# pc2/StencilStream

Measured on NVIDIA B200. Metric: GCell-updates/s, higher is better.
Workload: dtype f32

## Files before the change

include/stst_workloads.h:

```cpp
#ifndef STST_WORKLOADS_H
#define STST_WORKLOADS_H

#include <stddef.h>
#include <stdint.h>

#ifdef __cplusplus
extern "C" {
#endif

#define STST_WORKLOADS_ABI_VERSION 3

#define STST_OK 0
#define STST_ERR_UNKNOWN_WORKLOAD (-1)
#define STST_ERR_INVALID_ARGUMENT (-2)
#define STST_ERR_RANGE (-3)
#define STST_ERR_RUNTIME (-4)



typedef struct stst_hotspot_cell {
    float temp;
    float power;
} stst_hotspot_cell;

// ... 108 lines not shown
int stst_grid_max_abs(stst_grid *grid, const stst_field_extent *extents, size_t n, double *out);
int stst_grid_copy_field_to_host(stst_grid *grid, size_t field, void *values, size_t bytes);
int stst_grid_copy_field_from_host(stst_grid *grid, size_t field, const void *values, size_t bytes);


typedef struct stst_update stst_update;

typedef struct stst_update_params {
    const void *transition_function;
    size_t transition_function_bytes;
    const void *halo_value;
    size_t halo_value_bytes;
    size_t iteration_offset;
    size_t n_iterations;
    int blocking;
    int profiling;
    int cuda_device;
    unsigned fused_iterations;
    unsigned tile_rows;
    const int *cuda_devices;
    size_t n_cuda_devices;
} stst_update_params;

typedef struct stst_update_stats {
    size_t n_processed_cells;
    double walltime;
    double kernel_runtime;
    size_t n_launches;
    unsigned fused_iterations, tile_h, tile_w, block_x, block_y, use_tma;
    size_t smem_bytes;
    unsigned passthrough_planes;
    size_t speculation_redos;
    size_t n_slabs;
} stst_update_stats;

int stst_update_create(const char *workload, const stst_update_params *params, stst_update **update);
int stst_update_set_params(stst_update *update, const stst_update_params *params);
int stst_update_apply(stst_update *update, stst_grid *source, stst_grid **result);
int stst_update_get_stats(stst_update *update, stst_update_stats *stats);
int stst_update_destroy(stst_update *update);


typedef struct stst_slab stst_slab;

typedef struct stst_slab_info {
    size_t grid_rows, grid_cols, row_lo, row_hi;
    size_t ghost_rows;
    size_t device_bytes;
    size_t n_launches;
    size_t epoch;
    int device;
    unsigned fused_iterations, tile_h, tile_w, block_x, block_y, use_tma, overlap;
    size_t smem_bytes;
    unsigned passthrough_planes;
} stst_slab_info;

int stst_slab_create(const char *workload, size_t grid_rows, size_t grid_cols, size_t row_lo,
                     size_t row_hi, int device, unsigned fused_iterations, unsigned tile_rows,
                     int overlap, stst_slab **slab);
int stst_slab_destroy(stst_slab *slab);
int stst_slab_get_info(stst_slab *slab, stst_slab_info *info);
int stst_slab_get_ipc_handle(stst_slab *slab, unsigned char handle[64]);
int stst_slab_attach_ipc(stst_slab *slab, int side, const unsigned char handle[64],
                         size_t peer_row_lo, size_t peer_row_hi);
int stst_slab_attach_local(stst_slab *slab, int side, stst_slab *peer);
int stst_slab_use_nccl(stst_slab *slab, void *nccl_comm, int up_rank, int down_rank);
int stst_slab_detach(stst_slab *slab);
// ... 25 lines not shown
```

stencilstream_b200/_native.py:

```python
from __future__ import annotations

import ctypes as C
import os
from pathlib import Path

import numpy as np

PKG = Path(__file__).resolve().parent


class NativeLibraryMissing(RuntimeError):
    pass



class ConwayParams(C.Structure):
    _fields_ = [("reserved", C.c_int32)]


class Jacobi5Params(C.Structure):
    _fields_ = [("coef", C.c_float * 5)]


class Jacobi9Params(C.Structure):
# ... 28 lines not shown

class ConvectionThermalParams(C.Structure):
    _fields_ = [("nx", C.c_uint64), ("ny", C.c_uint64), ("dx", C.c_double), ("dy", C.c_double),
                ("dt", C.c_double), ("DcT", C.c_double)]


class KatParams(C.Structure):
    _fields_ = [("reserved", C.c_int32)]


class WorkloadInfo(C.Structure):
    _fields_ = [("cell_bytes", C.c_size_t), ("params_bytes", C.c_size_t), ("n_planes", C.c_size_t),
                ("stencil_radius", C.c_size_t), ("n_subiterations", C.c_size_t),
                ("bytes_per_cell_iteration", C.c_size_t)]


class UpdateParams(C.Structure):
    _fields_ = [
        ("transition_function", C.c_void_p), ("transition_function_bytes", C.c_size_t),
        ("halo_value", C.c_void_p), ("halo_value_bytes", C.c_size_t),
        ("iteration_offset", C.c_size_t), ("n_iterations", C.c_size_t),
        ("blocking", C.c_int), ("profiling", C.c_int), ("cuda_device", C.c_int),
        ("fused_iterations", C.c_uint), ("tile_rows", C.c_uint),
        ("cuda_devices", C.POINTER(C.c_int)), ("n_cuda_devices", C.c_size_t),
    ]


class UpdateStats(C.Structure):
    _fields_ = [
        ("n_processed_cells", C.c_size_t), ("walltime", C.c_double), ("kernel_runtime", C.c_double),
        ("n_launches", C.c_size_t), ("fused_iterations", C.c_uint), ("tile_h", C.c_uint),
        ("tile_w", C.c_uint), ("block_x", C.c_uint), ("block_y", C.c_uint), ("use_tma", C.c_uint),
        ("smem_bytes", C.c_size_t), ("passthrough_planes", C.c_uint), ("speculation_redos", C.c_size_t),
        ("n_slabs", C.c_size_t),
    ]


class FieldExtent(C.Structure):
    _fields_ = [("field", C.c_size_t), ("rows", C.c_size_t), ("cols", C.c_size_t)]


class DeviceInfo(C.Structure):
    _fields_ = [
        ("sm_count", C.c_int), ("cc_major", C.c_int), ("cc_minor", C.c_int),
        ("max_smem_per_block_optin", C.c_int), ("max_smem_per_sm", C.c_int), ("l2_bytes", C.c_int),
        ("clock_khz", C.c_int), ("total_mem", C.c_size_t), ("free_mem", C.c_size_t),
        ("name", C.c_char * 128),
    ]



CELL_DTYPES = {
    "conway": np.dtype(np.bool_),
    "jacobi5": np.dtype(np.float32),
    "jacobi9": np.dtype(np.float32),
    "jacobi_r2": np.dtype(np.float32),
    "jacobi_r3": np.dtype(np.float32),
    "hotspot": np.dtype([("temp", "<f4"), ("power", "<f4")]),
    "fdtd": np.dtype([(n, "<f4") for n in ("ex", "ey", "hz", "hz_sum", "ca", "cb", "da", "db")]),
    "convection_pt": np.dtype([(n, "<f8") for n in (
        "T", "Pt", "Vx", "Vy", "tau_xx", "tau_yy", "sigma_xy", "dVxd_tau", "dVyd_tau", "ErrV", "ErrP")]),
    "kat": np.dtype([(n, "<i4") for n in ("r", "c", "i_iteration", "i_subiteration", "status")]),
}
CELL_DTYPES["convection_thermal"] = CELL_DTYPES["convection_pt"]
CELL_DTYPES["kat_r2"] = CELL_DTYPES["kat"]


# ... 137 lines not shown
```

stencilstream_b200/csrc/workloads/model.hpp:

```cpp
#pragma once
#include <StencilStream/cuda/StencilUpdate.hpp>
#include <StencilStream/cuda/internal/SlabUpdate.hpp>
#include <stst_workloads.h>

#include "functors.hpp"

#include <algorithm>
#include <cstring>
#include <memory>
#include <stdexcept>
#include <string>
#include <vector>

namespace stst_model {

using namespace stst_workloads;
namespace sc = stencil::cuda;

inline thread_local std::string g_error;

inline int report(int code, std::string message) {
    g_error = std::move(message);
    return code;
}
// ... 102 lines not shown

    UpdateHolder(const char *name, const stst_update_params &p)
        : update(std::make_unique<Update>(convert(p))) {
        workload = name;
    }

    void set_params(const stst_update_params &p) override { update->get_params() = convert(p); }

    GridBase *apply(GridBase &source) override {
        auto *typed = dynamic_cast<GridHolder<Cell> *>(&source);
        if (!typed)
            throw std::invalid_argument("grid belongs to a workload with a different cell type");
        sc::Grid<Cell> result = (*update)(typed->grid);
        return new GridHolder<Cell>(source.workload, result);
    }

    void stats(stst_update_stats &s) override {
        std::memset(&s, 0, sizeof(s));
        s.n_processed_cells = update->get_n_processed_cells();
        s.walltime = update->get_walltime();
        s.kernel_runtime = update->get_kernel_runtime();
        s.n_launches = update->get_n_launches();
        auto const &plan = update->get_last_plan();
        s.fused_iterations = plan.fused_iterations;
        s.tile_h = plan.tile_h;
        s.tile_w = plan.tile_w;
        s.block_x = plan.block_x;
        s.block_y = plan.block_y;
        s.use_tma = plan.use_tma ? 1u : 0u;
        s.smem_bytes = plan.smem_bytes;
        s.passthrough_planes = update->get_passthrough_planes();
        s.speculation_redos = update->get_n_speculation_redos();
        s.n_slabs = update->get_n_slabs();
    }
};

struct SlabBase {
    virtual ~SlabBase() = default;
    const char *workload = nullptr;
    std::vector<void *> ipc_mappings;
    virtual std::size_t cell_bytes() const = 0;
    virtual void info(stst_slab_info &out) = 0;
    virtual void *device_base() = 0;
    virtual int device() const = 0;
    virtual void attach(int side, void *mapped, std::size_t lo, std::size_t hi) = 0;
    virtual void detach() = 0;
    virtual void use_nccl(void *comm, int up_rank, int down_rank) = 0;
    virtual void upload(const void *cells, std::size_t first_row, std::size_t n_rows) = 0;
    virtual void download(void *cells, std::size_t first_row, std::size_t n_rows) = 0;
    virtual void exchange() = 0;
    virtual void max_abs(const stst_field_extent *extents, std::size_t n, double *out) = 0;
    virtual std::size_t field_bytes(std::size_t field) const = 0;
    virtual void download_field(std::size_t field, void *host, std::size_t first_row,
                                std::size_t n_rows) = 0;
    virtual void update(const stst_update_params &p) = 0;
    virtual void synchronize() = 0;
    virtual void record(void *event) = 0;
    virtual void copy_from(SlabBase &other) = 0;
    virtual sc::internal::PlaneSet current_planes() = 0;
    virtual std::size_t ghost() const = 0;
    virtual bool enable_speculation(bool on) = 0;
    virtual void backup() = 0;
    virtual void restore() = 0;
    virtual unsigned take_violations() = 0;
    virtual void drop_passthrough(unsigned planes) = 0;
};
// ... 149 lines not shown
```

stencilstream_b200/include/StencilStream/cuda/StencilUpdate.hpp:

```cpp
#pragma once
#include "../Concepts.hpp"
#include "../Stencil.hpp"
#include "Grid.hpp"
#include "internal/Helpers.hpp"
#include "internal/Launch.hpp"
#include "internal/PassThrough.hpp"
#include "internal/Planner.hpp"
#include "internal/Runtime.hpp"
#include "internal/SlabUpdate.hpp"
#include "internal/TileKernel.hpp"

#include <algorithm>
#include <chrono>
#include <cstdio>
#include <cstdlib>
#include <memory>
#include <string>
#include <vector>

namespace stencil {
namespace cuda {

template <concepts::TransitionFunction F, bool split_cell_structure = false> class StencilUpdate {
  public:
// ... 174 lines not shown
    }

    GridImpl run_passes(GridImpl &source, internal::LaunchPlan const &plan,
                        internal::Speculation const *spec, std::size_t iteration,
                        std::size_t n_iterations, bool source_is_scratch = false) {
        last_plan = plan;
        const std::size_t k = plan.fused_iterations;
        GridImpl swap_a = source.make_similar();
        GridImpl swap_b = source_is_scratch ? source
                          : (n_iterations > k) ? source.make_similar()
                                               : swap_a;
        swap_a.get_storage().allocate_device();
        swap_b.get_storage().allocate_device();
        lap("allocate scratch grids");

        GridImpl *pass_source = &source, *pass_target = &swap_a;
        while (n_iterations > 0) {
            const unsigned n_gens = unsigned(std::min(n_iterations, k));
            launch(plan, pass_source->get_storage(), pass_target->get_storage(), iteration, n_gens,
                   spec);
            iteration += n_gens;
            n_iterations -= n_gens;
            pass_source = pass_target;
            pass_target = (pass_target == &swap_a) ? &swap_b : &swap_a;
        }
        pass_source->get_storage().device_written();
        lap("submit launches");
        return *pass_source;
    }

    internal::LaunchPlan plan_for(internal::GridStorage<Cell> const &source, unsigned single_planes) {
        const internal::LaunchPlan plan = internal::make_plan<F>(
            source.device, unsigned(source.height), unsigned(source.width), params.n_iterations,
            params.fused_iterations, params.tile_rows, single_planes);
        lap("make_plan");
        return plan;
    }

    void lap(const char *what) {
        if (!std::getenv("STST_TRACE"))
            return;
        const auto now = std::chrono::high_resolution_clock::now();
        std::fprintf(stderr, "[stst] %-22s %9.3f ms\n", what,
                     std::chrono::duration<double, std::milli>(now - lap_start).count());
        lap_start = now;
    }


    using Slab = internal::SlabUpdate<F>;

    struct ShardSet {
        ~ShardSet() {
            for (auto &slab : slabs)
                if (slab)
                    slab->synchronize();
        }
        std::vector<int> devices;
        std::size_t grid_h = 0, grid_w = 0;
        unsigned fused_override = 0, tile_rows = 0;
        std::vector<std::unique_ptr<Slab>> slabs;
        std::vector<std::unique_ptr<internal::Event>> done;
        bool speculating = false;
    };

    std::vector<int> resolve_devices() const {
        if (!params.cuda_devices.empty())
            return params.cuda_devices;
// ... 236 lines not shown
```

stencilstream_b200/include/StencilStream/cuda/internal/Launch.hpp:

```cpp
#pragma once
#include "Helpers.hpp"
#include "PassThrough.hpp"
#include "Planner.hpp"
#include "Runtime.hpp"
#include "TileKernel.hpp"

#include <climits>
#include <cstring>
#include <map>
#include <stdexcept>
#include <string>
#include <tuple>

namespace stencil {
namespace cuda {
namespace internal {

struct LaunchRegion {
    int device;
    unsigned grid_h, grid_w;
    int buf_row0;
    std::size_t buf_rows;
    int out_row_lo;
    int out_row_hi;
// ... 5 lines not shown
template <typename Cell> class TensorMapCache {
  public:
    using Layout = CellLayout<Cell>;

    TensorMapSet const &get(PlaneSet const &planes, std::size_t width, std::size_t rows,
                            unsigned box_cols, unsigned box_rows) {
        const Key key{planes.base[0], planes.pitch[0], width, rows, box_cols, box_rows};
        auto it = cache.find(key);
        if (it != cache.end())
            return it->second;
        if (cache.size() >= 64)
            cache.clear();
        TensorMapSet maps{};
        for (std::size_t i = 0; i < Layout::n_planes; i++) {
            STST_RT_CHECK(stst_tensor_map_encode_2d(
                &maps.map[i][0], planes.base[i], int(Layout::plane_bytes(i)), width, rows,
                planes.pitch[i] * Layout::plane_bytes(i), box_cols, box_rows));
        }
        return cache.emplace(key, maps).first->second;
    }

    void clear() { cache.clear(); }

  private:
    using Key = std::tuple<void *, unsigned long long, std::size_t, std::size_t, unsigned, unsigned>;
    std::map<Key, TensorMapSet> cache;
};

template <typename F> struct SweepLauncher {
    using Cell = typename F::Cell;
    using TDV = typename F::TimeDependentValue;
    using Layout = CellLayout<Cell>;
    static constexpr int CW = column_group_width<Cell>();
#if defined(STST_WINDOW_MODE)
    static constexpr int kMode = STST_WINDOW_MODE;
#else
    static constexpr int kMode = sizeof(Cell) <= 8    ? window_rotate
                                 : sizeof(Cell) <= 16 ? window_shift
                                                      : window_reload;
#endif

    static void launch(LaunchPlan const &plan, F const &tf, Cell const &halo_value,
                       PlaneSet const &src, PlaneSet const &dst, HaloPush const *push,
                       LaunchRegion const &region, std::size_t iteration0, unsigned n_gens,
                       TensorMapCache<Cell> &maps_cache, stst_stream_t stream,
                       Speculation const *spec = nullptr) {
#if defined(__CUDACC__)
        constexpr unsigned n_sub = unsigned(F::n_subiterations);
        constexpr unsigned radius = unsigned(F::stencil_radius);
        if (n_gens == 0 || n_gens > plan.fused_iterations || n_gens > max_fused_iterations)
            throw std::invalid_argument("StencilStream-B200: illegal number of fused iterations");
        if (region.out_row_hi <= region.out_row_lo || region.grid_w == 0)
            return;

        SweepGeometry geo{};
        geo.grid_h = region.grid_h;
        geo.grid_w = region.grid_w;
        geo.buf_row0 = region.buf_row0;
        geo.buf_rows = unsigned(region.buf_rows);
        geo.out_row_lo = region.out_row_lo;
        geo.out_row_hi = region.out_row_hi;
        geo.tile_h = region.tile_h ? std::min(region.tile_h, plan.tile_h) : plan.tile_h;
        const bool second = region.out2_row_hi > region.out2_row_lo;
        geo.tile_h = std::min(geo.tile_h, unsigned(region.out_row_hi - region.out_row_lo));
        if (second)
            geo.tile_h = std::min(geo.tile_h, unsigned(region.out2_row_hi - region.out2_row_lo));
        geo.tile_w = plan.tile_w;
        geo.halo = n_gens * n_sub * radius;
        geo.hpad = plan.hpad;
        geo.n_gens = n_gens;
        geo.tiles_x = (geo.grid_w + geo.tile_w - 1) / geo.tile_w;
        geo.use_tma = plan.use_tma ? 1u : 0u;
        geo.push = push ? 1u : 0u;
        geo.inv_block_y = (1u << 24) / plan.block_y + 1u;
        constexpr unsigned all_planes =
            Layout::n_planes >= 32 ? ~0u : ((1u << Layout::n_planes) - 1u);
        unsigned single_planes = 0;
        if (spec) {
            if constexpr (speculation_capable<F>()) {
                for (unsigned q = 0; q < n_sub && q < max_spec_subiterations; q++)
                    geo.keep[q] = spec->probe ? 0u : (spec->keep[q] & all_planes);
                geo.probe = spec->probe ? 1u : 0u;
                geo.spec_flags = spec->flags;
                single_planes = spec->probe ? 0u : spec->single_planes(n_sub, all_planes);
                if (single_planes != plan.single_planes)
                    throw std::logic_error("StencilStream-B200: plan and speculation masks disagree");
// ... 47 lines not shown
                                             cudaGetErrorString(err));
                configured_smem = smem;
            }
            kernel<<<grid, block, smem, static_cast<cudaStream_t>(stream)>>>(
                tf, halo_value, tdvs, src, dst, push ? *push : no_push, *maps, geo);
        };
        static std::size_t configured_smem_per_device[2][64] = {};
        if constexpr (speculation_capable<F>()) {
            if (spec) {
                submit(fused_sweep_kernel<F, CW, kMode, fixed_block_x<Cell>(),
                                          max_threads_per_cta<Cell>(), 1, true>,
                       configured_smem_per_device[1][region.device & 63]);
            } else {
                submit(fused_sweep_kernel<F, CW, kMode, fixed_block_x<Cell>(),
                                          max_threads_per_cta<Cell>(), 1, false>,
                       configured_smem_per_device[0][region.device & 63]);
            }
        } else {
            submit(fused_sweep_kernel<F, CW, kMode, fixed_block_x<Cell>(),
                                      max_threads_per_cta<Cell>(), 1, false>,
                   configured_smem_per_device[0][region.device & 63]);
        }
        cudaError_t err = cudaGetLastError();
        if (err != cudaSuccess)
            throw std::runtime_error(std::string("StencilStream-B200: kernel launch failed: ") +
                                     cudaGetErrorString(err));
#else
        (void)plan, (void)tf, (void)halo_value, (void)src, (void)dst, (void)push, (void)region;
        (void)iteration0, (void)n_gens, (void)maps_cache, (void)stream;
        throw std::runtime_error("StencilStream-B200 must be compiled with nvcc for sm_100a; "
                                 "there is no CPU fallback");
#endif
    }
};

}
}
}
```

stencilstream_b200/include/StencilStream/cuda/internal/Planner.hpp:

```cpp
#pragma once
#include "Helpers.hpp"
#include "Runtime.hpp"
#include "TileKernel.hpp"

#include <algorithm>
#include <cmath>
#include <cstdlib>
#include <stdexcept>
#include <string>

namespace stencil {
namespace cuda {
namespace internal {

struct LaunchPlan {
    unsigned fused_iterations;
    unsigned block_x, block_y;
    unsigned tile_h, tile_w;
    unsigned halo, hpad;
    std::size_t smem_bytes;
    bool use_tma;
    unsigned single_planes;
};

inline long env_long(const char *name, long fallback) {
    const char *v = std::getenv(name);
    return (v && *v) ? std::atol(v) : fallback;
}

inline const stst_device_info &cached_device_info(int device) {
    constexpr int max_devices = 64;
    static stst_device_info infos[max_devices];
    static bool valid[max_devices] = {};
    if (device < 0 || device >= max_devices)
        throw std::invalid_argument("StencilStream-B200: device ordinal out of range");
    if (!valid[device]) {
        STST_RT_CHECK(stst_get_device_info(device, &infos[device]));
        valid[device] = true;
    }
    return infos[device];
}

template <typename Cell> constexpr int column_group_width() {
    if (sizeof(Cell) > 64) {
#if defined(STST_FAT_COLUMN_GROUP_WIDTH)
        return STST_FAT_COLUMN_GROUP_WIDTH;
#else
        return 1;
#endif
    }
    const std::size_t widest = CellLayout<Cell>::max_plane_bytes();
    if (widest >= 16)
        return 1;
    if (widest >= 8)
        return 2;
// ... 5 lines not shown
#endif
    }
#if defined(STST_LIGHT_COLUMN_GROUP_WIDTH)
    if (CellLayout<Cell>::n_planes == 1 && widest == 4)
        return STST_LIGHT_COLUMN_GROUP_WIDTH;
#endif
    return 4;
}

template <typename Cell> constexpr int max_threads_per_cta() {
#if defined(STST_LIGHT_MAX_THREADS)
    if (sizeof(Cell) <= 8)
        return STST_LIGHT_MAX_THREADS;
#endif
    if (sizeof(Cell) > 16 && sizeof(Cell) <= 64) {
#if defined(STST_MID_MAX_THREADS)
        return STST_MID_MAX_THREADS;
#else
        return 384;
#endif
    }
    if (sizeof(Cell) > 64 && column_group_width<Cell>() == 1) {
#if defined(STST_FAT_MAX_THREADS)
        return STST_FAT_MAX_THREADS;
#else
        return 640;
#endif
    }
    return 256;
}

template <typename Cell> constexpr int fixed_block_x() {
    return lane_major_tiles<Cell, column_group_width<Cell>()>() ? 256 / column_group_width<Cell>() : 0;
}

template <typename Cell> constexpr bool tma_capable() {
    using L = CellLayout<Cell>;
    constexpr int cw = column_group_width<Cell>();
    for (std::size_t i = 0; i < L::n_planes; i++) {
        const std::size_t b = L::plane_bytes(i);
        if (!(b == 1 || b == 2 || b == 4 || b == 8))
            return false;
        if ((b * cw * 32) % 16 != 0)
            return false;
    }
    return true;
}

template <typename Cell> constexpr unsigned column_alignment(bool for_tma) {
    using L = CellLayout<Cell>;
    unsigned align = unsigned(column_group_width<Cell>());
    if (for_tma) {
        for (std::size_t i = 0; i < L::n_planes; i++) {
            const unsigned need = unsigned(16 / (L::plane_bytes(i) < 16 ? L::plane_bytes(i) : 16));
            align = need > align ? need : align;
        }
    }
    return align;
}

struct TileShape {
    unsigned halo, hpad, tile_h, tile_w, rows, cols;
    std::size_t smem_bytes;
    double efficiency;
    bool feasible;
};

template <typename Cell>
TileShape shape_for(unsigned k, unsigned n_sub, unsigned radius, unsigned cw, unsigned col_align,
                    unsigned block_x, unsigned tile_rows_override, std::size_t smem_budget,
                    unsigned grid_h, unsigned single_planes = 0) {
    TileShape s{};
    s.halo = k * n_sub * radius;
    s.hpad = (s.halo + col_align - 1) / col_align * col_align;
    s.cols = block_x * cw;
    s.feasible = false;
    if (2 * s.hpad >= s.cols)
        return s;
    s.tile_w = s.cols - 2 * s.hpad;
    const unsigned n_buffers = (k * n_sub > 1) ? 2 : 1;
    const std::size_t per_row = tile_buffer_bytes<Cell>(1, s.cols) +
                                tile_buffer_bytes<Cell>(1, s.cols, single_planes) * (n_buffers - 1);
    const std::size_t usable = smem_budget > 4096 ? smem_budget - 2048 : 0;
    unsigned max_rows = unsigned(std::min<std::size_t>(usable / std::max<std::size_t>(per_row, 1), 256));
    if (max_rows <= 2 * s.halo)
        return s;
    unsigned tile_h = max_rows - 2 * s.halo;
    if (tile_rows_override > 0)
        tile_h = std::min(tile_h, tile_rows_override);
    tile_h = std::min(tile_h, std::max(grid_h, 1u));
    s.tile_h = tile_h;
    s.rows = tile_h + 2 * s.halo;
    s.smem_bytes = tile_smem_bytes<Cell>(s.rows, s.cols, n_buffers, single_planes);
    s.efficiency = double(s.tile_h) * s.tile_w / (double(s.rows) * s.cols);
    s.feasible = s.smem_bytes <= smem_budget;
    return s;
}

template <typename F>
LaunchPlan make_plan(int device, unsigned grid_h, unsigned grid_w, std::size_t n_iterations,
                     unsigned fused_override, unsigned tile_rows_override,
                     unsigned single_planes = 0) {
    using Cell = typename F::Cell;
    using L = CellLayout<Cell>;
    constexpr unsigned cw = unsigned(column_group_width<Cell>());
    constexpr unsigned n_sub = unsigned(F::n_subiterations);
    constexpr unsigned radius = unsigned(F::stencil_radius);

    const stst_device_info &info = cached_device_info(device);
    const std::size_t smem_optin = std::size_t(info.max_smem_per_block_optin);
    const std::size_t smem_sm = std::size_t(info.max_smem_per_sm);

    unsigned block_x = unsigned(env_long("STST_BLOCK_X", 0));
    if (block_x == 0) {
        block_x = (sizeof(Cell) <= 16 || cw == 1) ? 64 : 32;
        if (cw > 4)
            block_x = 32;
        while (block_x > 32 && block_x * cw / 2 >= std::max(grid_w, 1u) + 2 * cw)
            block_x /= 2;
    }
    block_x = std::max(32u, block_x / 32 * 32);
    if (fixed_block_x<Cell>() != 0)
        block_x = unsigned(fixed_block_x<Cell>());
    unsigned block_y = unsigned(env_long("STST_BLOCK_Y", 0));
    if (block_y == 0)
        block_y = std::max(1u, unsigned(max_threads_per_cta<Cell>()) / block_x);
    if (block_x * block_y > unsigned(max_threads_per_cta<Cell>()))
        throw std::invalid_argument("StencilStream-B200: CTA shape exceeds the compiled thread limit");

    if (fused_override == 0)
        fused_override = unsigned(env_long("STST_FUSE", 0));
    if (tile_rows_override == 0)
        tile_rows_override = unsigned(env_long("STST_TILE_ROWS", 0));
    const unsigned ctas_per_sm = unsigned(std::max(1l, env_long("STST_CTAS_PER_SM", 2)));

    const unsigned k_cap = unsigned(
        std::min<std::size_t>(std::max<std::size_t>(n_iterations, 1), max_fused_iterations));

    auto budget_for = [&](unsigned ctas) {
        std::size_t per_cta = smem_sm / ctas;
        per_cta = per_cta > 1024 ? per_cta - 1024 : 0;
        return std::min(per_cta, smem_optin);
    };

    const bool want_tma = tma_capable<Cell>() && env_long("STST_TMA", 1) != 0;
    const unsigned col_align = column_alignment<Cell>(want_tma);

    auto evaluate = [&](unsigned k, unsigned ctas) {
        return shape_for<Cell>(k, n_sub, radius, cw, col_align, block_x, tile_rows_override,
                               budget_for(ctas), grid_h, single_planes);
    };

    unsigned best_k = 0;
    TileShape best{};
    const double hbm_bytes = 2.0 * double(sizeof(Cell)) * n_sub;
    const double onchip = (0.475 * double(sizeof(Cell)) * n_sub + 0.4 * n_sub) *
                          (1.0 + 0.28 * double(radius - 1));
    if (fused_override > 0) {
        for (unsigned k = std::min(fused_override, k_cap); k >= 1 && best_k == 0; k--) {
            double best_cost = 0.0;
            for (unsigned ctas : {ctas_per_sm, 1u}) {
                const TileShape s = evaluate(k, ctas);
                if (!s.feasible)
                    continue;
                const double solo = (ctas == 1 && ctas_per_sm > 1) ? 1.40 : 1.0;
                const double hbm = hbm_bytes / k;
                const double cost = solo * std::sqrt(hbm * hbm + onchip * onchip) / s.efficiency;
                if (best_k == 0 || cost < best_cost) {
                    best_k = k;
                    best = s;
// ... 26 lines not shown
                break;
        }
        if (best_k == 0)
            throw std::invalid_argument(
                "StencilStream-B200: cell type too large for a shared-memory tile");
    }

    if (tile_rows_override == 0 && best.tile_h > 2 * best.halo) {
        const unsigned tiles_x = (std::max(grid_w, 1u) + best.tile_w - 1) / best.tile_w;
        const unsigned slots = unsigned(std::max(info.sm_count, 1)) * ctas_per_sm;
        const unsigned want_tile_rows = std::max(1u, slots * 95u / 100u / tiles_x);
        const unsigned tile_h =
            std::max(2 * best.halo, (std::max(grid_h, 1u) + want_tile_rows - 1) / want_tile_rows);
        if (tile_h < best.tile_h) {
            const TileShape shrunk =
                shape_for<Cell>(best_k, n_sub, radius, cw, col_align, block_x, tile_h,
                                budget_for(ctas_per_sm), grid_h, single_planes);
            if (shrunk.feasible)
                best = shrunk;
        }
    }

    LaunchPlan plan{};
    plan.fused_iterations = best_k;
    plan.block_x = block_x;
    plan.block_y = block_y;
    plan.tile_h = best.tile_h;
    plan.tile_w = best.tile_w;
    plan.halo = best.halo;
    plan.hpad = best.hpad;
    plan.smem_bytes = best.smem_bytes;
    plan.use_tma = want_tma && best.cols <= 256 && best.rows <= 256;
    plan.single_planes = single_planes;
    (void)L::n_planes;
    return plan;
}

}
}
}
```

stencilstream_b200/include/StencilStream/cuda/internal/SlabUpdate.hpp:

```cpp
#pragma once
#include "FieldOps.hpp"
#include "Helpers.hpp"
#include "Launch.hpp"
#include "PassThrough.hpp"
#include "Planner.hpp"
#include "Runtime.hpp"
#include "TileKernel.hpp"

#include <algorithm>
#include <climits>
#include <cstdint>
#include <cstdlib>
#include <memory>
#include <stdexcept>
#include <string>
#include <vector>

namespace stencil {
namespace cuda {
namespace internal {

#if defined(__CUDACC__)
template <int = 0> __global__ void raise_flag_kernel(volatile unsigned *flag, unsigned value) {
    __threadfence_system();
// ... 39 lines not shown
        }
        return set;
    }

    static unsigned *flag(void *base, int which) { return static_cast<unsigned *>(base) + which; }
};

inline void partition_rows(std::size_t rows, std::size_t count, std::size_t index, std::size_t &lo,
                           std::size_t &hi) {
    const std::size_t base = rows / count, extra = rows % count;
    lo = index * base + std::min(index, extra);
    hi = lo + base + (index < extra ? 1 : 0);
}

enum class SlabSide : int { up = 0, down = 1 };

template <typename F> class SlabUpdate {
  public:
    using Cell = typename F::Cell;
    using Layout = CellLayout<Cell>;

    struct Config {
        std::size_t grid_rows, grid_cols;
        std::size_t row_lo, row_hi;
        int device;
        unsigned fused_iterations;
        unsigned tile_rows;
        bool overlap;
    };

    explicit SlabUpdate(Config const &config)
        : cfg(config), plan(make_plan<F>(config.device, unsigned(config.row_hi - config.row_lo),
                                         unsigned(config.grid_cols), max_fused_iterations,
                                         config.fused_iterations, config.tile_rows)),
          ghost(std::size_t(plan.fused_iterations) * F::n_subiterations * F::stencil_radius),
          layout(config.grid_cols, config.row_hi - config.row_lo, ghost), base(nullptr), epoch(0),
          n_launches(0), interior_stream(nullptr), boundary_stream(nullptr) {
        if (cfg.row_hi <= cfg.row_lo || cfg.row_hi > cfg.grid_rows)
            throw std::invalid_argument("StencilStream-B200: illegal slab row range");
        if (cfg.grid_rows > 0x7fffffffull || cfg.grid_cols > 0x7fffffffull)
            throw std::range_error("StencilStream-B200 grids are limited to 2^31-1 rows/columns");
        const bool has_neighbour = cfg.row_lo > 0 || cfg.row_hi < cfg.grid_rows;
        if (has_neighbour && owned_rows() < ghost)
            throw std::invalid_argument(
                "StencilStream-B200: a slab must own at least k*n_sub*radius rows (its neighbour's "
                "ghost rows must come from one slab); use fewer GPUs or a smaller fused_iterations");
        STST_RT_CHECK(stst_set_device(cfg.device));
        boundary_done = std::make_unique<Event>();
        interior_done = std::make_unique<Event>();
        STST_RT_CHECK(stst_malloc_ipc(cfg.device, layout.total_bytes, &base));
        STST_RT_CHECK(stst_stream_create(cfg.device, 0, &interior_stream));
        STST_RT_CHECK(stst_stream_create(cfg.device, 1, &boundary_stream));
        STST_RT_CHECK(stst_memset_async(base, 0, SlabLayout<Cell>::flag_bytes, interior_stream));
        STST_RT_CHECK(stst_stream_synchronize(interior_stream));
        for (int s = 0; s < 2; s++) {
            peer_base[s] = nullptr;
            peer_row_lo[s] = peer_row_hi[s] = 0;
        }
        if (PassThrough<F>::declared())
            plan_passthrough();
    }

    SlabUpdate(SlabUpdate const &) = delete;
    SlabUpdate &operator=(SlabUpdate const &) = delete;

    ~SlabUpdate() {
        (void)stst_stream_synchronize(interior_stream);
// ... 286 lines not shown
        select_device();
        raise_flag_kernel<><<<1, 1, 0, static_cast<cudaStream_t>(boundary_stream)>>>(peer_flag(s),
                                                                                     value);
        if (cudaGetLastError() != cudaSuccess)
            throw std::runtime_error("StencilStream-B200: flag kernel launch failed");
        n_launches++;
#else
        (void)s, (void)value;
        throw std::runtime_error("StencilStream-B200 must be compiled with nvcc for sm_100a");
#endif
    }

    void select_device() {
#if defined(__CUDACC__)
        int current = -1;
        if (cudaGetDevice(&current) != cudaSuccess || current != cfg.device)
            cudaSetDevice(cfg.device);
#endif
    }

    void join_streams() {
        select_device();
        boundary_done->record(boundary_stream);
        STST_RT_CHECK(stst_stream_wait_event(interior_stream, boundary_done->get()));
        interior_done->record(interior_stream);
        STST_RT_CHECK(stst_stream_wait_event(boundary_stream, interior_done->get()));
    }

    void fork_streams() { join_streams(); }

    void plan_passthrough() {
        spec_plan = make_plan<F>(cfg.device, unsigned(cfg.row_hi - cfg.row_lo),
                                 unsigned(cfg.grid_cols), max_fused_iterations,
                                 plan.fused_iterations, cfg.tile_rows, pass_through.single_planes());
        if (spec_plan.fused_iterations != plan.fused_iterations)
            throw std::logic_error("StencilStream-B200: pass-through changed the fusion depth");
    }

    std::size_t plane_set_bytes() const {
        return layout.plane_offset[1][0] - layout.plane_offset[0][0];
    }
    unsigned char *plane_set_begin(int buffer) const {
        return static_cast<unsigned char *>(base) + layout.plane_offset[buffer][0];
    }

    void pass(F const &tf, Cell const &halo_value, std::size_t iteration0, unsigned n_gens,
              Speculation const *spec) {
        const LaunchPlan &use_plan = (spec && !spec->probe) ? spec_plan : plan;
        const int cur = int(epoch & 1);
        const PlaneSet src = layout.planes(base, cur);
        const PlaneSet dst = layout.planes(base, cur ^ 1);

        HaloPush push{};
        push.up_row_hi = INT_MIN;
        push.down_row_lo = INT_MAX;
        for (int s = 0; s < 2 && !nccl_comm; s++) {
            if (!has_side(s))
                continue;
            require_attached(s);
            const SlabLayout<Cell> peer(cfg.grid_cols, peer_row_hi[s] - peer_row_lo[s], ghost);
            const PlaneSet theirs = peer.planes(peer_base[s], cur ^ 1);
            if (s == 0) {
                push.up = theirs;
                push.up_buf_row0 = int(peer_row_lo[s]) - int(ghost);
                push.up_row_hi = int(cfg.row_lo + ghost);
            } else {
                push.down = theirs;
// ... 169 lines not shown
```

stencilstream_b200/include/StencilStream/cuda/internal/TileKernel.hpp:

```cpp
#pragma once
#include "../../Stencil.hpp"
#include "Helpers.hpp"

#include <cuda_runtime.h>

#include <cstddef>
#include <cstdint>
#include <type_traits>

namespace stencil {
namespace cuda {
namespace internal {

inline constexpr int store_tile = 0, store_grid = 1, store_runtime = 2;

template <typename Cell, int CW> constexpr bool lane_major_tiles() {
#if defined(STST_NO_LANE_MAJOR)
    return false;
#else
    using L = CellLayout<Cell>;
    if (!(CW == 4 || CW == 8))
        return false;
    const unsigned constant = constant_fields_mask<Cell>();
    unsigned evolving = 0;
// ... 1025 lines not shown
        const Cell cell = aos[idx];
        for_each_plane<Cell>([&](auto I) {
            using T = typename L::template plane_t<I>;
            static_cast<T *>(planes.base[I])[(plane_row0 + r) * planes.pitch[I] + c] =
                L::template get<I>(cell);
        });
    }
}

template <typename Cell>
__global__ void __launch_bounds__(256)
    gather_cells_kernel(Cell *__restrict__ aos, PlaneSet planes, unsigned long long width,
                        unsigned long long plane_row0, unsigned long long n_cells) {
    using L = CellLayout<Cell>;
    const unsigned long long stride = (unsigned long long)gridDim.x * blockDim.x;
    for (unsigned long long idx = (unsigned long long)blockIdx.x * blockDim.x + threadIdx.x;
         idx < n_cells; idx += stride) {
        const unsigned long long r = idx / width, c = idx - r * width;
        Cell cell;
        for_each_plane<Cell>([&](auto I) {
            using T = typename L::template plane_t<I>;
            L::template get<I>(cell) =
                static_cast<const T *>(planes.base[I])[(plane_row0 + r) * planes.pitch[I] + c];
        });
        aos[idx] = cell;
    }
}

#endif

}
}
}
```

Measured before the change: 2026.

## Add warp-streaming temporal-blocking kernel for single-plane f32 radius-1 stencils

Adds a new streaming kernel in which each warp sweeps a 128-column strip down a row segment, fed by a 4-stage TMA ring of 3-row stages per warp. It fuses up to six iterations using rotating register row windows, so halo rows are recomputed only at segment ends instead of around full 2D tiles. A cost model chooses fusion depth and segment height from SM count, occupancy and a simple issue/HBM bound. The path is used automatically for eligible functors in the single-grid update, but not for slabs. This adds a lot of new code and relies on an untested cost model.

```diff
diff --git a/include/stst_workloads.h b/include/stst_workloads.h
--- a/include/stst_workloads.h
+++ b/include/stst_workloads.h
@@ -164,7 +164,11 @@
     unsigned passthrough_planes;
     size_t speculation_redos;
     size_t n_slabs;
+    unsigned kernel;
 } stst_update_stats;
+
+#define STST_KERNEL_TILE 0
+#define STST_KERNEL_STREAM 1
 
 int stst_update_create(const char *workload, const stst_update_params *params, stst_update **update);
 int stst_update_set_params(stst_update *update, const stst_update_params *params);
diff --git a/stencilstream_b200/_native.py b/stencilstream_b200/_native.py
--- a/stencilstream_b200/_native.py
+++ b/stencilstream_b200/_native.py
@@ -84,7 +84,7 @@
         ("n_launches", C.c_size_t), ("fused_iterations", C.c_uint), ("tile_h", C.c_uint),
         ("tile_w", C.c_uint), ("block_x", C.c_uint), ("block_y", C.c_uint), ("use_tma", C.c_uint),
         ("smem_bytes", C.c_size_t), ("passthrough_planes", C.c_uint), ("speculation_redos", C.c_size_t),
-        ("n_slabs", C.c_size_t),
+        ("n_slabs", C.c_size_t), ("kernel", C.c_uint),
     ]
 
 
diff --git a/stencilstream_b200/csrc/workloads/model.hpp b/stencilstream_b200/csrc/workloads/model.hpp
--- a/stencilstream_b200/csrc/workloads/model.hpp
+++ b/stencilstream_b200/csrc/workloads/model.hpp
@@ -158,6 +158,7 @@
         s.passthrough_planes = update->get_passthrough_planes();
         s.speculation_redos = update->get_n_speculation_redos();
         s.n_slabs = update->get_n_slabs();
+        s.kernel = plan.kernel;
     }
 };
 
diff --git a/stencilstream_b200/include/StencilStream/cuda/StencilUpdate.hpp b/stencilstream_b200/include/StencilStream/cuda/StencilUpdate.hpp
--- a/stencilstream_b200/include/StencilStream/cuda/StencilUpdate.hpp
+++ b/stencilstream_b200/include/StencilStream/cuda/StencilUpdate.hpp
@@ -230,7 +230,7 @@
     internal::LaunchPlan plan_for(internal::GridStorage<Cell> const &source, unsigned single_planes) {
         const internal::LaunchPlan plan = internal::make_plan<F>(
             source.device, unsigned(source.height), unsigned(source.width), params.n_iterations,
-            params.fused_iterations, params.tile_rows, single_planes);
+            params.fused_iterations, params.tile_rows, single_planes, true);
         lap("make_plan");
         return plan;
     }
diff --git a/stencilstream_b200/include/StencilStream/cuda/internal/Launch.hpp b/stencilstream_b200/include/StencilStream/cuda/internal/Launch.hpp
--- a/stencilstream_b200/include/StencilStream/cuda/internal/Launch.hpp
+++ b/stencilstream_b200/include/StencilStream/cuda/internal/Launch.hpp
@@ -61,13 +61,7 @@
     using TDV = typename F::TimeDependentValue;
     using Layout = CellLayout<Cell>;
     static constexpr int CW = column_group_width<Cell>();
-#if defined(STST_WINDOW_MODE)
-    static constexpr int kMode = STST_WINDOW_MODE;
-#else
-    static constexpr int kMode = sizeof(Cell) <= 8    ? window_rotate
-                                 : sizeof(Cell) <= 16 ? window_shift
-                                                      : window_reload;
-#endif
+    static constexpr int kMode = window_mode<Cell>();
 
     static void launch(LaunchPlan const &plan, F const &tf, Cell const &halo_value,
                        PlaneSet const &src, PlaneSet const &dst, HaloPush const *push,
@@ -81,6 +75,18 @@
             throw std::invalid_argument("StencilStream-B200: illegal number of fused iterations");
         if (region.out_row_hi <= region.out_row_lo || region.grid_w == 0)
             return;
+        if (plan.kernel == plan_stream) {
+            if constexpr (streamable<F>()) {
+                if (push || spec || region.out2_row_hi > region.out2_row_lo)
+                    throw std::logic_error("StencilStream-B200: a streaming plan covers one row range "
+                                           "of one grid, without halo push or pass-through");
+                launch_stream(plan, tf, halo_value, src, dst, region, iteration0, n_gens, maps_cache,
+                              stream);
+                return;
+            } else {
+                throw std::logic_error("StencilStream-B200: streaming plan for a tile-only functor");
+            }
+        }
 
         SweepGeometry geo{};
         geo.grid_h = region.grid_h;
@@ -194,6 +200,57 @@
                                  "there is no CPU fallback");
 #endif
     }
+
+#if defined(__CUDACC__)
+    static void launch_stream(LaunchPlan const &plan, F const &tf, Cell const &halo_value,
+                              PlaneSet const &src, PlaneSet const &dst, LaunchRegion const &region,
+                              std::size_t iteration0, unsigned n_gens,
+                              TensorMapCache<Cell> &maps_cache, stst_stream_t stream) {
+        if (n_gens > stream_max_depth || plan.hpad < n_gens)
+            throw std::invalid_argument("StencilStream-B200: illegal depth of a streaming launch");
+        StreamGeometry geo{};
+        geo.grid_h = region.grid_h;
+        geo.grid_w = region.grid_w;
+        geo.buf_row0 = region.buf_row0;
+        geo.out_row_lo = region.out_row_lo;
+        geo.out_row_hi = region.out_row_hi;
+        geo.seg_rows = plan.tile_h;
+        geo.strip_w = plan.tile_w;
+        geo.hpad = plan.hpad;
+        geo.strips = (geo.grid_w + geo.strip_w - 1) / geo.strip_w;
+        const unsigned segments =
+            (unsigned(region.out_row_hi - region.out_row_lo) + geo.seg_rows - 1) / geo.seg_rows;
+        geo.items = geo.strips * segments;
+        geo.iteration0 = iteration0;
+
+        TdvArray<TDV> tdvs{};
+        for (unsigned g = 0; g < n_gens; g++)
+            tdvs.v[g] = tf.get_time_dependent_value(iteration0 + g);
+        TensorMapSet const &maps = maps_cache.get(src, region.grid_w, region.buf_rows,
+                                                  stream_strip_cols, stream_stage_rows);
+
+        int current_device = -1;
+        if (cudaGetDevice(&current_device) != cudaSuccess || current_device != region.device) {
+            if (cudaSetDevice(region.device) != cudaSuccess)
+                throw std::runtime_error("StencilStream-B200: cannot select CUDA device " +
+                                         std::to_string(region.device));
+        }
+        const dim3 block(stream_warps * 32, 1, 1);
+        const dim3 grid((geo.items + stream_warps - 1) / stream_warps, 1, 1);
+        const std::size_t smem = stream_smem_bytes();
+        auto submit = [&](auto kernel) {
+            kernel<<<grid, block, smem, static_cast<cudaStream_t>(stream)>>>(tf, halo_value, tdvs, dst,
+                                                                             maps, geo);
+        };
+        [&]<unsigned... Ds>(std::integer_sequence<unsigned, Ds...>) {
+            ((n_gens == Ds + 1 ? submit(stream_sweep_kernel<F, Ds + 1>) : void()), ...);
+        }(std::make_integer_sequence<unsigned, stream_max_depth>{});
+        cudaError_t err = cudaGetLastError();
+        if (err != cudaSuccess)
+            throw std::runtime_error(std::string("StencilStream-B200: kernel launch failed: ") +
+                                     cudaGetErrorString(err));
+    }
+#endif
 };
 
 }
diff --git a/stencilstream_b200/include/StencilStream/cuda/internal/Planner.hpp b/stencilstream_b200/include/StencilStream/cuda/internal/Planner.hpp
--- a/stencilstream_b200/include/StencilStream/cuda/internal/Planner.hpp
+++ b/stencilstream_b200/include/StencilStream/cuda/internal/Planner.hpp
@@ -12,6 +12,8 @@
 namespace stencil {
 namespace cuda {
 namespace internal {
+
+inline constexpr unsigned plan_tile = 0, plan_stream = 1;
 
 struct LaunchPlan {
     unsigned fused_iterations;
@@ -21,6 +23,7 @@
     std::size_t smem_bytes;
     bool use_tma;
     unsigned single_planes;
+    unsigned kernel;
 };
 
 inline long env_long(const char *name, long fallback) {
@@ -92,6 +95,19 @@
 
 template <typename Cell> constexpr int fixed_block_x() {
     return lane_major_tiles<Cell, column_group_width<Cell>()>() ? 256 / column_group_width<Cell>() : 0;
+}
+
+template <typename Cell> constexpr int window_mode() {
+#if defined(STST_WINDOW_MODE)
+    return STST_WINDOW_MODE;
+#else
+    return sizeof(Cell) <= 8 ? window_rotate : sizeof(Cell) <= 16 ? window_shift : window_reload;
+#endif
+}
+
+template <typename F> constexpr bool streamable() {
+    using Cell = typename F::Cell;
+    return streamed_sweeps<F, column_group_width<Cell>(), window_mode<Cell>(), false>();
 }
 
 template <typename Cell> constexpr bool tma_capable() {
@@ -157,10 +173,62 @@
     return s;
 }
 
+inline LaunchPlan make_stream_plan(unsigned sm_count, unsigned warps_per_sm, unsigned grid_h,
+                                   unsigned grid_w, unsigned k_min, unsigned k_max,
+                                   unsigned rows_override) {
+    constexpr double c_gen = 5.0, c_row = 10.0;
+    constexpr double issue_per_cycle = 128 * 0.55;
+    constexpr double bytes_per_cycle = 23.0;
+    const unsigned resident = std::max(1u, sm_count * warps_per_sm);
+    const unsigned h = std::max(grid_h, 1u), w = std::max(grid_w, 1u);
+    static constexpr unsigned candidates[] = {16, 24, 32, 48, 64, 96, 128, 192, 256, 384,
+                                              512, 768, 1024, 1536, 2048};
+    double best_cost = 0.0;
+    LaunchPlan plan{};
+    for (unsigned k = std::max(k_min, 1u); k <= std::min(k_max, stream_max_depth); k++) {
+        const unsigned hpad = (k + stream_cw - 1) / stream_cw * stream_cw;
+        const unsigned strip_w = stream_strip_cols - 2 * hpad;
+        const unsigned strips = (w + strip_w - 1) / strip_w;
+        const double eff_h = double(strip_w) / stream_strip_cols;
+        auto consider = [&](unsigned S) {
+            S = std::min(S, h);
+            const unsigned segments = (h + S - 1) / S;
+            const double items = double(strips) * segments;
+            const double waves = std::ceil(items / resident);
+            const double eff_v = double(S) / (S + 2.0 * k);
+            const double issue = (c_gen + c_row / k) / issue_per_cycle / (eff_h * eff_v);
+            const double hbm = (4.0 / (eff_h * eff_v) + 4.0) / k / bytes_per_cycle;
+            const double cost = std::sqrt(issue * issue + hbm * hbm) /
+                                (items / (waves * resident)) * (1.0 + 0.5 / waves);
+            if (plan.fused_iterations == 0 || cost < best_cost * 0.995) {
+                best_cost = cost;
+                plan.fused_iterations = k;
+                plan.tile_h = S;
+                plan.tile_w = strip_w;
+                plan.halo = k;
+                plan.hpad = hpad;
+            }
+        };
+        if (rows_override > 0) {
+            consider(rows_override);
+        } else {
+            for (unsigned S : candidates)
+                consider(S);
+        }
+    }
+    plan.block_x = 32;
+    plan.block_y = stream_warps;
+    plan.smem_bytes = stream_smem_bytes();
+    plan.use_tma = true;
+    plan.single_planes = 0;
+    plan.kernel = plan_stream;
+    return plan;
+}
+
 template <typename F>
 LaunchPlan make_plan(int device, unsigned grid_h, unsigned grid_w, std::size_t n_iterations,
                      unsigned fused_override, unsigned tile_rows_override,
-                     unsigned single_planes = 0) {
+                     unsigned single_planes = 0, bool allow_stream = false) {
     using Cell = typename F::Cell;
     using L = CellLayout<Cell>;
     constexpr unsigned cw = unsigned(column_group_width<Cell>());
@@ -196,6 +264,22 @@
 
     const unsigned k_cap = unsigned(
         std::min<std::size_t>(std::max<std::size_t>(n_iterations, 1), max_fused_iterations));
+
+    if constexpr (streamable<F>()) {
+        const long stream = env_long("STST_STREAM", -1);
+        const bool automatic = fused_override == 0 && tile_rows_override == 0;
+        if (allow_stream && single_planes == 0 && stream != 0 && (stream == 1 || automatic)) {
+            const StreamKernelInfo kernel = stream_kernel_info<F>();
+            const unsigned k_max =
+                std::min(fused_override > 0 ? std::min(fused_override, k_cap) : k_cap,
+                         kernel.max_depth);
+            const unsigned rows = tile_rows_override > 0
+                                      ? tile_rows_override
+                                      : unsigned(std::max(0l, env_long("STST_STREAM_ROWS", 0)));
+            return make_stream_plan(unsigned(std::max(info.sm_count, 1)), kernel.warps_per_sm,
+                                    grid_h, grid_w, fused_override > 0 ? k_max : 1, k_max, rows);
+        }
+    }
 
     auto budget_for = [&](unsigned ctas) {
         std::size_t per_cta = smem_sm / ctas;
@@ -288,6 +372,7 @@
     plan.smem_bytes = best.smem_bytes;
     plan.use_tma = want_tma && best.cols <= 256 && best.rows <= 256;
     plan.single_planes = single_planes;
+    plan.kernel = plan_tile;
     (void)L::n_planes;
     return plan;
 }
diff --git a/stencilstream_b200/include/StencilStream/cuda/internal/SlabUpdate.hpp b/stencilstream_b200/include/StencilStream/cuda/internal/SlabUpdate.hpp
--- a/stencilstream_b200/include/StencilStream/cuda/internal/SlabUpdate.hpp
+++ b/stencilstream_b200/include/StencilStream/cuda/internal/SlabUpdate.hpp
@@ -95,7 +95,8 @@
     explicit SlabUpdate(Config const &config)
         : cfg(config), plan(make_plan<F>(config.device, unsigned(config.row_hi - config.row_lo),
                                          unsigned(config.grid_cols), max_fused_iterations,
-                                         config.fused_iterations, config.tile_rows)),
+                                         config.fused_iterations, config.tile_rows, 0,
+                                         false)),
           ghost(std::size_t(plan.fused_iterations) * F::n_subiterations * F::stencil_radius),
           layout(config.grid_cols, config.row_hi - config.row_lo, ghost), base(nullptr), epoch(0),
           n_launches(0), interior_stream(nullptr), boundary_stream(nullptr) {
@@ -448,7 +449,8 @@
     void plan_passthrough() {
         spec_plan = make_plan<F>(cfg.device, unsigned(cfg.row_hi - cfg.row_lo),
                                  unsigned(cfg.grid_cols), max_fused_iterations,
-                                 plan.fused_iterations, cfg.tile_rows, pass_through.single_planes());
+                                 plan.fused_iterations, cfg.tile_rows, pass_through.single_planes(),
+                                 false);
         if (spec_plan.fused_iterations != plan.fused_iterations)
             throw std::logic_error("StencilStream-B200: pass-through changed the fusion depth");
     }
diff --git a/stencilstream_b200/include/StencilStream/cuda/internal/StreamKernel.hpp b/stencilstream_b200/include/StencilStream/cuda/internal/StreamKernel.hpp
--- /dev/null
+++ b/stencilstream_b200/include/StencilStream/cuda/internal/StreamKernel.hpp
@@ -0,0 +1,287 @@
+#pragma once
+#include "TileKernel.hpp"
+
+namespace stencil {
+namespace cuda {
+namespace internal {
+
+inline constexpr unsigned stream_max_depth = 6;
+inline constexpr unsigned stream_cw = 4;
+inline constexpr unsigned stream_strip_cols = 128;
+inline constexpr unsigned stream_stage_rows = 3;
+inline constexpr unsigned stream_stages = 4;
+inline constexpr unsigned stream_warps = 4;
+inline constexpr unsigned stream_stage_bytes = stream_stage_rows * stream_strip_cols * 4;
+
+STST_HD constexpr std::size_t stream_smem_bytes() {
+    return std::size_t(stream_warps) * stream_stages * stream_stage_bytes;
+}
+
+template <typename F, int CW, int kMode, bool kSpec> constexpr bool streamed_sweeps() {
+    using L = CellLayout<typename F::Cell>;
+    return L::n_planes == 1 && sizeof(typename F::Cell) == 4 && L::plane_bytes(0) == 4 &&
+           CW == int(stream_cw) && F::stencil_radius == 1 && F::n_subiterations == 1 &&
+           kMode == window_rotate && !kSpec;
+}
+
+struct StreamGeometry {
+    unsigned grid_h, grid_w;
+    int buf_row0;
+    int out_row_lo, out_row_hi;
+    unsigned seg_rows;
+    unsigned strip_w;
+    unsigned hpad;
+    unsigned strips;
+    unsigned items;
+    unsigned long long iteration0;
+};
+
+#if defined(__CUDACC__)
+
+template <typename F, unsigned N, bool kColMask, bool kRowTest>
+__device__ __forceinline__ void
+stream_segment(F const &tf, typename F::Cell const &halo_value,
+               TdvArray<typename F::TimeDependentValue> const &tdvs, PlaneSet const &dst,
+               TensorMapSet const &maps, StreamGeometry const &geo, unsigned char *ring,
+               unsigned long long *bar, int y0, int rows_out, int gx_in0, int lane) {
+    using Cell = typename F::Cell;
+    using TDV = typename F::TimeDependentValue;
+    using StencilImpl = Stencil<Cell, 1, TDV>;
+    constexpr int CW = int(stream_cw), WW = CW + 2;
+    constexpr int NST = int(stream_stages), SR = int(stream_stage_rows);
+    static_assert(SR == 3, "a stage holds one rotation of the row windows");
+
+    const int n_steps = rows_out + 2 * int(N);
+    const int n_stages = (n_steps + SR - 1) / SR;
+    const int gy_in0 = y0 - int(N);
+    const int gx = gx_in0 + lane * CW;
+
+    auto issue = [&](int s) {
+        const int b = s % NST;
+        mbarrier_arrive_expect_tx(&bar[b], stream_stage_bytes);
+        tma_load_2d(ring + b * stream_stage_bytes, &maps.map[0][0], gx_in0,
+                    gy_in0 + s * SR - geo.buf_row0, &bar[b]);
+    };
+    if (lane == 0) {
+        for (int s = 0; s < NST && s < n_stages; s++)
+            issue(s);
+    }
+
+    bool col_in[CW];
+#pragma unroll
+    for (int i = 0; i < CW; i++)
+        col_in[i] = !kColMask || (gx + i >= 0 && gx + i < int(geo.grid_w));
+    const bool own = lane * CW >= int(geo.hpad) && lane * CW < int(stream_strip_cols - geo.hpad);
+
+    Cell w[N][3][WW];
+    unsigned stage = 0;
+
+    auto put_row = [&](Cell(&row)[WW], Cell const (&v)[CW]) {
+#pragma unroll
+        for (int i = 0; i < CW; i++)
+            row[1 + i] = v[i];
+        row[0] = shuffle_from_lower_lane(v[CW - 1]);
+        row[CW + 1] = shuffle_from_upper_lane(v[0]);
+    };
+
+    const long long pitch = (long long)dst.pitch[0];
+    Cell *out = static_cast<Cell *>(dst.base[0]) + (long long)(y0 - geo.buf_row0) * pitch + gx;
+    auto store_row = [&](Cell const (&v)[CW]) {
+        Cell *g = out;
+        out += pitch;
+        if (!own)
+            return;
+        if (!kColMask || gx + CW <= int(geo.grid_w)) {
+            Pack<Cell, CW> q;
+#pragma unroll
+            for (int i = 0; i < CW; i++)
+                q.v[i] = v[i];
+            *reinterpret_cast<Pack<Cell, CW> *>(g) = q;
+        } else {
+#pragma unroll
+            for (int i = 0; i < CW; i++)
+                if (gx + i < int(geo.grid_w))
+                    g[i] = v[i];
+        }
+    };
+
+    auto step = [&](auto p_c, auto ng_c, int t, auto test_c) {
+        constexpr int P = decltype(p_c)::value;
+        constexpr int NG = decltype(ng_c)::value;
+        constexpr bool kTest = kRowTest && decltype(test_c)::value;
+        const unsigned b = stage % NST;
+        if constexpr (P == 0)
+            mbarrier_wait_parity(&bar[b], (stage / NST) & 1u);
+        const Pack<Cell, CW> p = *reinterpret_cast<const Pack<Cell, CW> *>(
+            ring + b * stream_stage_bytes + P * stream_strip_cols * 4 + lane * CW * 4);
+        if constexpr (P == SR - 1) {
+            __syncwarp();
+            if (lane == 0 && int(stage) + NST < n_stages) {
+                fence_proxy_async();
+                issue(int(stage) + NST);
+            }
+            stage++;
+        }
+        Cell v[CW];
+        {
+            const bool row_in = !kTest || unsigned(gy_in0 + t) < geo.grid_h;
+#pragma unroll
+            for (int i = 0; i < CW; i++)
+                v[i] = (row_in && col_in[i]) ? p.v[i] : halo_value;
+        }
+        put_row(w[0][P], v);
+
+#pragma unroll
+        for (int g = 1; g <= NG; g++) {
+            const int gy = gy_in0 + t - g;
+            const int top = ((P - g - 1) % 3 + 3) % 3;
+            const std::size_t it = std::size_t(geo.iteration0) + std::size_t(g - 1);
+            const bool row_in = !kTest || unsigned(gy) < geo.grid_h;
+            Cell r[CW];
+#pragma unroll
+            for (int i = 0; i < CW; i++) {
+                const std::size_t id_r = std::size_t(unsigned(gy)), id_c = std::size_t(unsigned(gx + i));
+                const std::size_t range_r = geo.grid_h, range_c = geo.grid_w;
+                if constexpr (!kRowTest) {
+                    __builtin_assume(id_r != 0);
+                    __builtin_assume(id_r != range_r - 1);
+                    __builtin_assume(id_r < range_r - 1);
+                    __builtin_assume(id_r + 1 < range_r);
+                }
+                if constexpr (!kColMask) {
+                    __builtin_assume(id_c != 0);
+                    __builtin_assume(id_c != range_c - 1);
+                    __builtin_assume(id_c < range_c - 1);
+                    __builtin_assume(id_c + 1 < range_c);
+                }
+                StencilImpl st(sycl::id<2>(id_r, id_c), sycl::range<2>(range_r, range_c), it, 0,
+                               tdvs.v[g - 1]);
+#pragma unroll
+                for (int sr = 0; sr < 3; sr++) {
+#pragma unroll
+                    for (int sc = 0; sc < 3; sc++)
+                        st[sycl::id<2>(sr, sc)] = w[g - 1][(top + sr) % 3][i + sc];
+                }
+                const Cell c = tf(st);
+                r[i] = (row_in && col_in[i]) ? c : halo_value;
+            }
+            if (g < int(N))
+                put_row(w[g < int(N) ? g : 0][((P - g) % 3 + 3) % 3], r);
+            else
+                store_row(r);
+        }
+    };
+
+    using test = std::true_type;
+    using no_test = std::false_type;
+
+    [&]<int... Ts>(std::integer_sequence<int, Ts...>) {
+        (step(int_c<Ts % 3>{}, int_c<(Ts / 2 < int(N) ? Ts / 2 : int(N))>{}, Ts, test{}), ...);
+    }(std::make_integer_sequence<int, 2 * int(N)>{});
+
+    constexpr int P0 = (2 * int(N)) % 3;
+    const int untested_end =
+        kRowTest ? min(n_steps, int(geo.grid_h) - y0 + int(N)) : n_steps;
+    int t = 2 * int(N);
+    for (; t + 3 <= untested_end; t += 3) {
+        step(int_c<P0>{}, int_c<int(N)>{}, t, no_test{});
+        step(int_c<(P0 + 1) % 3>{}, int_c<int(N)>{}, t + 1, no_test{});
+        step(int_c<(P0 + 2) % 3>{}, int_c<int(N)>{}, t + 2, no_test{});
+    }
+    if constexpr (kRowTest) {
+        for (; t + 3 <= n_steps; t += 3) {
+            step(int_c<P0>{}, int_c<int(N)>{}, t, test{});
+            step(int_c<(P0 + 1) % 3>{}, int_c<int(N)>{}, t + 1, test{});
+            step(int_c<(P0 + 2) % 3>{}, int_c<int(N)>{}, t + 2, test{});
+        }
+    }
+    if (t < n_steps) {
+        step(int_c<P0>{}, int_c<int(N)>{}, t, test{});
+        if (t + 1 < n_steps)
+            step(int_c<(P0 + 1) % 3>{}, int_c<int(N)>{}, t + 1, test{});
+    }
+}
+
+template <typename F, unsigned N>
+__global__ void __launch_bounds__(stream_warps * 32, 4)
+    stream_sweep_kernel(const __grid_constant__ F tf,
+                        const __grid_constant__ typename F::Cell halo_value,
+                        const __grid_constant__ TdvArray<typename F::TimeDependentValue> tdvs,
+                        const __grid_constant__ PlaneSet dst,
+                        const __grid_constant__ TensorMapSet maps,
+                        const __grid_constant__ StreamGeometry geo) {
+    extern __shared__ __align__(128) unsigned char smem[];
+    __shared__ unsigned long long bars[stream_warps][stream_stages];
+
+    const int warp = int(threadIdx.x) / 32, lane = int(threadIdx.x) & 31;
+    const unsigned item = blockIdx.x * stream_warps + unsigned(warp);
+    if (item >= geo.items)
+        return;
+    const unsigned seg = item / geo.strips, strip = item - seg * geo.strips;
+    const int y0 = geo.out_row_lo + int(seg * geo.seg_rows);
+    const int rows_out = min(int(geo.seg_rows), geo.out_row_hi - y0);
+    const int gx_in0 = int(strip * geo.strip_w) - int(geo.hpad);
+
+    unsigned long long *bar = bars[warp];
+    if (lane == 0) {
+#pragma unroll
+        for (unsigned s = 0; s < stream_stages; s++)
+            mbarrier_init(&bar[s], 1);
+        fence_mbarrier_init();
+    }
+    __syncwarp();
+    unsigned char *ring = smem + std::size_t(warp) * stream_stages * stream_stage_bytes;
+
+    const bool rows_inside = y0 >= int(N) && y0 + rows_out + int(N) <= int(geo.grid_h);
+    const bool cols_inside = gx_in0 >= 1 && gx_in0 + int(stream_strip_cols) + 1 <= int(geo.grid_w);
+    if (rows_inside && cols_inside)
+        stream_segment<F, N, false, false>(tf, halo_value, tdvs, dst, maps, geo, ring, bar, y0,
+                                           rows_out, gx_in0, lane);
+    else if (cols_inside)
+        stream_segment<F, N, false, true>(tf, halo_value, tdvs, dst, maps, geo, ring, bar, y0,
+                                          rows_out, gx_in0, lane);
+    else
+        stream_segment<F, N, true, true>(tf, halo_value, tdvs, dst, maps, geo, ring, bar, y0,
+                                         rows_out, gx_in0, lane);
+}
+
+#endif
+
+struct StreamKernelInfo {
+    unsigned max_depth;
+    unsigned warps_per_sm;
+};
+
+template <typename F> StreamKernelInfo stream_kernel_info() {
+#if defined(__CUDACC__)
+    static const StreamKernelInfo info = [] {
+        StreamKernelInfo result{1, 16};
+        bool spilled = false;
+        [&]<unsigned... Ds>(std::integer_sequence<unsigned, Ds...>) {
+            auto probe = [&](unsigned depth, auto kernel) {
+                cudaFuncAttributes attr{};
+                int ctas = 0;
+                spilled = spilled || cudaFuncGetAttributes(&attr, kernel) != cudaSuccess ||
+                          attr.localSizeBytes != 0 ||
+                          cudaOccupancyMaxActiveBlocksPerMultiprocessor(
+                              &ctas, kernel, int(stream_warps * 32), stream_smem_bytes()) !=
+                              cudaSuccess ||
+                          ctas < 1;
+                if (spilled)
+                    return;
+                result.max_depth = depth;
+                result.warps_per_sm = unsigned(ctas) * stream_warps;
+            };
+            (probe(Ds + 1, stream_sweep_kernel<F, Ds + 1>), ...);
+        }(std::make_integer_sequence<unsigned, stream_max_depth>{});
+        return result;
+    }();
+    return info;
+#else
+    return {stream_max_depth, 16};
+#endif
+}
+
+}
+}
+}
diff --git a/stencilstream_b200/include/StencilStream/cuda/internal/TileKernel.hpp b/stencilstream_b200/include/StencilStream/cuda/internal/TileKernel.hpp
--- a/stencilstream_b200/include/StencilStream/cuda/internal/TileKernel.hpp
+++ b/stencilstream_b200/include/StencilStream/cuda/internal/TileKernel.hpp
@@ -1081,3 +1081,5 @@
 }
 }
 }
+
+#include "StreamKernel.hpp"
```

After: 3263 (median of 6 runs). 1.61x the previous value.
